# CityU-AIM-Group/SimT

Hardware: AMD Instinct MI355X
Metric: training images/sec at 768x768, DeepLabv2-R101+SimT (higher is better)
Workload: dtype bf16; 1 GPU; DeepLabv2-ResNet101 + SimT(C=19,K=3) full training iteration, batch=4/GPU, 768x768, bf16, 1xMI355X; global_batch=4, inputs=resident in HBM (see h2d_inclusive of a --full run for the PCIe-inclusive rate)

## Files before the change

### simt_amd/csrc/bn_pool.hip

```cpp
#include "common.h"

template <int NJ>
__device__ __forceinline__ void part_colsum8(const float* part, int nblk, int C, int c0, double* out , double (*red)[8][NJ]) {
  const int cl = threadIdx.x & 7, r = threadIdx.x >> 3;
  const int c = c0 + cl;
  double s[NJ];
#pragma unroll
  for (int j = 0; j < NJ; ++j) s[j] = 0.0;
  if (c < C) {
    int b = r;
    for (; b + 96 < nblk; b += 128) {
      float v[4][NJ];
#pragma unroll
      for (int u = 0; u < 4; ++u)
#pragma unroll
        for (int j = 0; j < NJ; ++j) v[u][j] = part[((long)(b + 32 * u) * NJ + j) * C + c];
#pragma unroll
      for (int u = 0; u < 4; ++u)
#pragma unroll
        for (int j = 0; j < NJ; ++j) s[j] += (double)v[u][j];
    }
    for (; b < nblk; b += 32)
#pragma unroll
      for (int j = 0; j < NJ; ++j) s[j] += (double)part[((long)b * NJ + j) * C + c];
// ... 308 lines not shown
      gr[u] = *(const uint2*)(dzb + ou);
      yr[u] = *(const uint2*)(yb + ou);
      if (MM == 1) zr[u] = *(const uint2*)(zb + ou);
      if (MM == 3) bb[u] = (unsigned)((const unsigned char*)zb)[ou >> 4] >> ((ou >> 1) & 4u);
    }
#pragma unroll
    for (int u = 0; u < UN; ++u) {
      const unsigned ou = o0 + u * Sb;
      if (ou >= nb) break;
      float g[4], yv[4];
      unpack4(gr[u], g);
      unpack4(yr[u], yv);
      if (MM == 1) {
        float zv[4];
        unpack4(zr[u], zv);
#pragma unroll
        for (int e = 0; e < 4; ++e) g[e] = zv[e] > 0.f ? g[e] : 0.f;
      } else if (MM == 2) {
#pragma unroll
        for (int e = 0; e < 4; ++e) g[e] = (yv[e] * sc[e] + sh[e]) > 0.f ? g[e] : 0.f;
      } else if (MM == 3) {
#pragma unroll
        for (int e = 0; e < 4; ++e) g[e] = ((bb[u] >> e) & 1u) ? g[e] : 0.f;
      }
      float o[4];
#pragma unroll
      for (int e = 0; e < 4; ++e) o[e] = sc[e] * (g[e] - c1[e] - ((yv[e] - mu[e]) * rs[e]) * c2[e]);
      *(uint2*)(dyb + ou) = make_uint2(pack_bf16x2(o[0], o[1]), pack_bf16x2(o[2], o[3]));
      if (gout) *(uint2*)(gb + ou) = make_uint2(pack_bf16x2(g[0], g[1]), pack_bf16x2(g[2], g[3]));
    }
  }
}

static inline int bn_bwd_rows_per_block(long M, int C) {
  int rpar = 256 / (C / 8);
  long target_blocks = 512;
  long rpb = (M + target_blocks - 1) / target_blocks;
  rpb = ((rpb + rpar - 1) / rpar) * rpar;
  if (rpb < rpar * 4) rpb = rpar * 4;
  return (int)rpb;
}

extern "C" int simt_bn_bwd_nblk(long M, int C) {
  int rpb = bn_bwd_rows_per_block(M, C);
  return (int)((M + rpb - 1) / rpb);
}

extern "C" int simt_bn_bwd(const simt_bn_bwd_desc* d, simt_stream_t stream) {
  SIMT_CHECK(d && d->dz && d->y && d->mean && d->rstd && d->scale && d->part && d->coef && d->dy);
  SIMT_CHECK(d->C % 8 == 0 && d->C / 8 <= 256 && 256 % (d->C / 8) == 0);
  SIMT_CHECK((d->mask_mode != 1 && d->mask_mode != 3) || d->z);
  SIMT_CHECK(d->mask_mode != 2 || d->shift);
  SIMT_CHECK(!d->y2 || (d->mean2 && d->rstd2 && d->scale2 && d->dy2));
  hipStream_t st = (hipStream_t)stream;
  const int rpb = bn_bwd_rows_per_block(d->M, d->C);
  const int nblk = d->reduce_done_nblk > 0 ? d->reduce_done_nblk : (int)((d->M + rpb - 1) / rpb);
  const long nvec = d->M * (d->C / 8);
  if (d->reduce_done_nblk > 0) {
    SIMT_CHECK(!d->y2);
  } else if (d->dtype == SIMT_BF16) {
    hipLaunchKernelGGL(bn_bwd_reduce_kernel<bf16_t>, dim3(nblk), dim3(256), 0, st, (const bf16_t*)d->dz,
                       (const bf16_t*)d->z, (const bf16_t*)d->y, d->mean, d->rstd, d->scale, d->shift,
                       (const bf16_t*)d->y2, d->mean2, d->rstd2, d->part, d->M, d->C, rpb, d->mask_mode);
  } else {
    hipLaunchKernelGGL(bn_bwd_reduce_kernel<float>, dim3(nblk), dim3(256), 0, st, (const float*)d->dz,
                       (const float*)d->z, (const float*)d->y, d->mean, d->rstd, d->scale, d->shift,
                       (const float*)d->y2, d->mean2, d->rstd2, d->part, d->M, d->C, rpb, d->mask_mode);
  }
  SIMT_LAUNCH_CHECK();
  hipLaunchKernelGGL(bn_bwd_finalize_kernel, dim3((d->C + 7) / 8), dim3(256), 0, st, d->part, nblk, d->C, d->M, d->coef,
                     d->dgamma, d->dbeta, d->dgamma2, d->dbeta2);
  SIMT_LAUNCH_CHECK();
  if (SIMT_BNB_APPLY4 && d->dtype == SIMT_BF16 && !d->y2 && nvec * 16 < (1l << 31)) {
#ifndef SIMT_BNB_APPLY4_CAP
#define SIMT_BNB_APPLY4_CAP 4096
#endif
    long gl = (nvec * 2 + 256l * SIMT_BNB_APPLY4_UN - 1) / (256l * SIMT_BNB_APPLY4_UN);
    int g4 = (int)(gl > SIMT_BNB_APPLY4_CAP ? SIMT_BNB_APPLY4_CAP : gl < 1 ? 1 : gl);
    if (d->C / 4 > 256) g4 = (g4 + 1) & ~1;
#define SIMT_BNB4(MM) hipLaunchKernelGGL(bn_bwd_apply4_kernel<MM>, dim3(g4), dim3(256), 0, st, (const bf16_t*)d->dz, (const bf16_t*)d->z, (const bf16_t*)d->y, \
                                         d->mean, d->rstd, d->scale, d->shift, d->coef, (bf16_t*)d->dy, (bf16_t*)d->gout, nvec * 2, d->C)
    if (d->mask_mode == 3) SIMT_BNB4(3); else if (d->mask_mode == 2) SIMT_BNB4(2); else if (d->mask_mode == 1) SIMT_BNB4(1); else SIMT_BNB4(0);
#undef SIMT_BNB4
  } else if (d->dtype == SIMT_BF16) {
    hipLaunchKernelGGL(bn_bwd_apply_kernel<bf16_t>, dim3(ew_grid(nvec)), dim3(256), 0, st, (const bf16_t*)d->dz,
                       (const bf16_t*)d->z, (const bf16_t*)d->y, d->mean, d->rstd, d->scale, d->shift, d->coef,
                       (const bf16_t*)d->y2, d->mean2, d->rstd2, d->scale2, (bf16_t*)d->dy, (bf16_t*)d->dy2,
                       (bf16_t*)d->gout, nvec, d->C, d->mask_mode);
  } else {
    hipLaunchKernelGGL(bn_bwd_apply_kernel<float>, dim3(ew_grid(nvec)), dim3(256), 0, st, (const float*)d->dz,
                       (const float*)d->z, (const float*)d->y, d->mean, d->rstd, d->scale, d->shift, d->coef,
                       (const float*)d->y2, d->mean2, d->rstd2, d->scale2, (float*)d->dy, (float*)d->dy2,
                       (float*)d->gout, nvec, d->C, d->mask_mode);
  }
  SIMT_LAUNCH_CHECK();
  return SIMT_OK;
}

template <typename T, int KHC, int KWC>
__global__ void im2col_stem_kernel(const float* x, T* A, int B, int Cin, int H, int W, int Ho, int Wo, int KHr, int KWr,
                                   int stride, int pad, int ldk, long nvec) {
  const int KH = KHC > 0 ? KHC : KHr, KW = KWC > 0 ? KWC : KWr;
  const int vpr = ldk >> 3;
  const int K = Cin * KH * KW;
  for (long i = (long)blockIdx.x * blockDim.x + threadIdx.x; i < nvec; i += (long)gridDim.x * blockDim.x) {
    int kv = (int)(i % vpr) << 3;
    long m = i / vpr;
    int ox = (int)(m % Wo);
    long t = m / Wo;
    int oy = (int)(t % Ho);
    int b = (int)(t / Ho);
    const int iy0 = oy * stride - pad, ix0 = ox * stride - pad;
    const float* xb = x + (long)b * Cin * H * W;
    float v[8];
#pragma unroll
    for (int e = 0; e < 8; ++e) {
      int k = kv + e;
      float val = 0.f;
      if (k < K) {
        int ci = k / (KH * KW);
        int rs = k - ci * KH * KW;
        int r = rs / KW, s = rs - r * KW;
        int iy = iy0 + r, ix = ix0 + s;
        if (iy >= 0 && iy < H && ix >= 0 && ix < W) val = xb[((long)ci * H + iy) * W + ix];
      }
      v[e] = val;
    }
    store8(A + i * 8, v);
  }
}

template <typename T>
static void launch_im2col(const float* x, T* A, int B, int Cin, int H, int W, int Ho, int Wo, int KH, int KW, int stride, int pad,
                          int ldk, long nvec, hipStream_t st) {
  const dim3 grid(ew_grid(nvec)), blk(256);
  if (KH == 7 && KW == 7)
    hipLaunchKernelGGL((im2col_stem_kernel<T, 7, 7>), grid, blk, 0, st, x, A, B, Cin, H, W, Ho, Wo, KH, KW, stride, pad, ldk, nvec);
  else if (KH == 3 && KW == 3)
    hipLaunchKernelGGL((im2col_stem_kernel<T, 3, 3>), grid, blk, 0, st, x, A, B, Cin, H, W, Ho, Wo, KH, KW, stride, pad, ldk, nvec);
  else
    hipLaunchKernelGGL((im2col_stem_kernel<T, 0, 0>), grid, blk, 0, st, x, A, B, Cin, H, W, Ho, Wo, KH, KW, stride, pad, ldk, nvec);
}

extern "C" int simt_im2col_stem(const float* x, void* A, int B, int Cin, int H, int W, int Ho, int Wo, int KH, int KW,
                                int stride, int pad, int ldk, int dtype, simt_stream_t stream) {
  SIMT_CHECK(x && A && ldk % 8 == 0 && ldk >= Cin * KH * KW);
  long nvec = (long)B * Ho * Wo * (ldk / 8);
  if (dtype == SIMT_BF16) launch_im2col<bf16_t>(x, (bf16_t*)A, B, Cin, H, W, Ho, Wo, KH, KW, stride, pad, ldk, nvec, (hipStream_t)stream);
  else launch_im2col<float>(x, (float*)A, B, Cin, H, W, Ho, Wo, KH, KW, stride, pad, ldk, nvec, (hipStream_t)stream);
  SIMT_LAUNCH_CHECK();
  return SIMT_OK;
}

template <typename T>
__global__ void bn_relu_maxpool_kernel(const T* y, const float* scale, const float* shift, T* p, unsigned char* idx,
                                       int B, int H, int W, int C, int Hp, int Wp, long nvec) {
  const int vpr = C >> 3;
  for (long i = (long)blockIdx.x * blockDim.x + threadIdx.x; i < nvec; i += (long)gridDim.x * blockDim.x) {
    int c = (int)(i % vpr) << 3;
    long m = i / vpr;
    int px = (int)(m % Wp);
    long t = m / Wp;
    int py = (int)(t % Hp);
    int b = (int)(t / Hp);
    float sc[8], sh[8], best[8];
    int bi[8];
    load8(scale + c, sc);
    load8(shift + c, sh);
#pragma unroll
    for (int e = 0; e < 8; ++e) { best[e] = -INFINITY; bi[e] = 0; }
    bool first = true;
    for (int r = 0; r < 3; ++r) {
      int iy = py * 2 - 1 + r;
      if (iy < 0 || iy >= H) continue;
      for (int s = 0; s < 3; ++s) {
        int ix = px * 2 - 1 + s;
        if (ix < 0 || ix >= W) continue;
        float v[8];
        load8(y + (((long)b * H + iy) * W + ix) * C + c, v);
#pragma unroll
        for (int e = 0; e < 8; ++e) {
          float a = v[e] * sc[e] + sh[e];
          a = a > 0.f ? a : 0.f;
          if (first || a > best[e] || a != a) { best[e] = a; bi[e] = r * 3 + s; }
        }
        first = false;
      }
    }
    store8(p + i * 8, best);
    unsigned long long packed = 0;
#pragma unroll
    for (int e = 0; e < 8; ++e) packed |= (unsigned long long)(bi[e] & 0xff) << (8 * e);
    *(unsigned long long*)(idx + i * 8) = packed;
  }
}

template <typename T>
__global__ void maxpool_bwd_kernel(const T* dp, const unsigned char* idx, T* da, int B, int H, int W, int C, int Hp,
                                   int Wp, long nvec) {
  const int vpr = C >> 3;
  for (long i = (long)blockIdx.x * blockDim.x + threadIdx.x; i < nvec; i += (long)gridDim.x * blockDim.x) {
    int c = (int)(i % vpr) << 3;
    long m = i / vpr;
    int ix = (int)(m % W);
    long t = m / W;
    int iy = (int)(t % H);
    int b = (int)(t / H);
    float acc[8];
#pragma unroll
    for (int e = 0; e < 8; ++e) acc[e] = 0.f;
    int py0 = iy >> 1, px0 = ix >> 1;
    for (int py = py0; py <= ((iy + 1) >> 1); ++py) {
      if (py >= Hp) continue;
      int r = iy - (py * 2 - 1);
      if (r < 0 || r > 2) continue;
      for (int px = px0; px <= ((ix + 1) >> 1); ++px) {
        if (px >= Wp) continue;
        int s = ix - (px * 2 - 1);
        if (s < 0 || s > 2) continue;
        long o = (((long)b * Hp + py) * Wp + px) * C + c;
        unsigned long long packed = *(const unsigned long long*)(idx + o);
        float g[8];
        load8(dp + o, g);
        int want = r * 3 + s;
#pragma unroll
        for (int e = 0; e < 8; ++e)
          if ((int)((packed >> (8 * e)) & 0xff) == want) acc[e] += g[e];
      }
    }
    store8(da + i * 8, acc);
  }
}

extern "C" int simt_bn_relu_maxpool(const void* y, const float* scale, const float* shift, void* p, unsigned char* idx,
                                    int B, int H, int W, int C, int Hp, int Wp, int dtype, simt_stream_t stream) {
  SIMT_CHECK(y && scale && shift && p && idx && C % 8 == 0);
  long nvec = (long)B * Hp * Wp * (C / 8);
  if (dtype == SIMT_BF16)
    hipLaunchKernelGGL(bn_relu_maxpool_kernel<bf16_t>, dim3(ew_grid(nvec)), dim3(256), 0, (hipStream_t)stream,
                       (const bf16_t*)y, scale, shift, (bf16_t*)p, idx, B, H, W, C, Hp, Wp, nvec);
  else
    hipLaunchKernelGGL(bn_relu_maxpool_kernel<float>, dim3(ew_grid(nvec)), dim3(256), 0, (hipStream_t)stream,
                       (const float*)y, scale, shift, (float*)p, idx, B, H, W, C, Hp, Wp, nvec);
  SIMT_LAUNCH_CHECK();
  return SIMT_OK;
}

extern "C" int simt_maxpool_bwd(const void* dp, const unsigned char* idx, void* da, int B, int H, int W, int C, int Hp,
                                int Wp, int dtype, simt_stream_t stream) {
  SIMT_CHECK(dp && idx && da && C % 8 == 0);
  long nvec = (long)B * H * W * (C / 8);
  if (dtype == SIMT_BF16)
    hipLaunchKernelGGL(maxpool_bwd_kernel<bf16_t>, dim3(ew_grid(nvec)), dim3(256), 0, (hipStream_t)stream,
                       (const bf16_t*)dp, idx, (bf16_t*)da, B, H, W, C, Hp, Wp, nvec);
  else
    hipLaunchKernelGGL(maxpool_bwd_kernel<float>, dim3(ew_grid(nvec)), dim3(256), 0, (hipStream_t)stream, (const float*)dp,
                       idx, (float*)da, B, H, W, C, Hp, Wp, nvec);
  SIMT_LAUNCH_CHECK();
  return SIMT_OK;
}

__device__ __forceinline__ long long frag_offset(long long row, long long kcol, int nt16) {
  const long long kt = kcol >> 6, s = (kcol >> 5) & 1, kq = (kcol >> 3) & 3, e = kcol & 7;
  const long long lane = (row & 15) | (kq << 4);
  return ((((kt * nt16 + (row >> 4)) * 2 + s) * 64 + lane) << 3) + e;
}
template <typename T>
__global__ void pack_weight_kernel(const float* w, T* dst, int Cout, int Cin, int RS, int row_off, int tap_off, long ldk,
                                   int Ck, int mode, const float* cscale, long total) {
  for (long i = (long)blockIdx.x * blockDim.x + threadIdx.x; i < total; i += (long)gridDim.x * blockDim.x) {
    int t = (int)(i % RS);
    long r = i / RS;
    int ci = (int)(r % Cin);
    int co = (int)(r / Cin);
    float v = w[i];
    if (cscale) v *= cscale[co];
    const int lm = mode & 0xff, nt16 = mode >> 8;
    const long row = lm == 0 ? (long)(row_off + co) : lm == 1 ? (long)ci : (long)(tap_off + t) * Ck + row_off + co;
    const long kcol = lm == 0 ? (long)(tap_off + t) * Cin + ci : lm == 1 ? (long)(tap_off + t) * Ck + row_off + co : (long)ci;
    const long o = nt16 ? (long)frag_offset(row, kcol, nt16) : row * ldk + kcol;
    Elem<T>::st(dst + o, v);
  }
}

extern "C" int simt_pack_weight(const float* w, void* dst, int Cout, int Cin, int RS, int row_off, int tap_off, long ldk,
                                int Ck, int mode, const float* cscale, int dtype, simt_stream_t stream) {
  SIMT_CHECK(w && dst && Cout > 0 && Cin > 0 && RS > 0);
  long total = (long)Cout * Cin * RS;
  if (dtype == SIMT_BF16)
    hipLaunchKernelGGL(pack_weight_kernel<bf16_t>, dim3(ew_grid(total)), dim3(256), 0, (hipStream_t)stream, w, (bf16_t*)dst,
                       Cout, Cin, RS, row_off, tap_off, ldk, Ck, mode, cscale, total);
  else
    hipLaunchKernelGGL(pack_weight_kernel<float>, dim3(ew_grid(total)), dim3(256), 0, (hipStream_t)stream, w, (float*)dst,
                       Cout, Cin, RS, row_off, tap_off, ldk, Ck, mode, cscale, total);
  SIMT_LAUNCH_CHECK();
  return SIMT_OK;
}

struct PackJob {
  const float* w;
  void* dst;
  const float* cscale;
  long long ldk, total;
  int Cout, Cin, RS, row_off, tap_off, Ck, mode, dtype;
};
template <int RSC>
__device__ __forceinline__ void pack_tile(const PackJob& j, int tidx, float* tile) {
  const int ntc = (j.Cin + 31) >> 5;
  const int co0 = (tidx / ntc) << 5, ci0 = (tidx % ntc) << 5;
  const int RS = RSC > 0 ? RSC : j.RS;
  const int nci = min(32, j.Cin - ci0), nco = min(32, j.Cout - co0);
  for (int tb = 0; tb < RS; tb += 9) {
    const int nt = min(9, RS - tb);
    __syncthreads();
    const int per_co = nci * RS;
    for (int e = threadIdx.x; e < nco * per_co; e += 256) {
      const int co_l = e / per_co, rem = e - co_l * per_co;
      const int ci_l = rem / RS, t = rem - ci_l * RS;
      if (t < tb || t >= tb + nt) continue;
      float v = j.w[((long long)(co0 + co_l) * j.Cin + ci0) * RS + rem];
      if (j.cscale) v *= j.cscale[co0 + co_l];
      tile[((t - tb) * 32 + co_l) * 33 + ci_l] = v;
    }
    __syncthreads();
    for (int e = threadIdx.x; e < nt * 32 * 32; e += 256) {
      const int t = e >> 10;
      int co_l, ci_l;
      const int lm = j.mode & 0xff, nt16 = j.mode >> 8;
      if (lm == 1) { co_l = e & 31; ci_l = (e >> 5) & 31; } else { ci_l = e & 31; co_l = (e >> 5) & 31; }
      if (co_l >= nco || ci_l >= nci) continue;
      const float v = tile[(t * 32 + co_l) * 33 + ci_l];
      const int co = co0 + co_l, ci = ci0 + ci_l, tt = j.tap_off + tb + t;
      const long long row = lm == 0 ? (long long)(j.row_off + co) : lm == 1 ? (long long)ci : (long long)tt * j.Ck + j.row_off + co;
      const long long kcol = lm == 0 ? (long long)tt * j.Cin + ci : lm == 1 ? (long long)tt * j.Ck + j.row_off + co : (long long)ci;
      const long long o = nt16 ? frag_offset(row, kcol, nt16) : row * j.ldk + kcol;
      if (j.dtype == SIMT_BF16) ((bf16_t*)j.dst)[o] = f2bf(v); else ((float*)j.dst)[o] = v;
    }
  }
}
__global__ __launch_bounds__(256) void pack_weight_multi_kernel(const PackJob* jobs, const int* chunks, int ) {
  __shared__ float tile[9 * 32 * 33];
  const PackJob j = jobs[chunks[2 * blockIdx.x]];
  const int tidx = chunks[2 * blockIdx.x + 1];
  if (j.RS == 1) pack_tile<1>(j, tidx, tile);
  else if (j.RS == 9) pack_tile<9>(j, tidx, tile);
  else pack_tile<0>(j, tidx, tile);
}
extern "C" int simt_pack_weight_multi(const void* jobs, const void* chunks, int nchunks, int chunk, simt_stream_t stream) {
  SIMT_CHECK(jobs && chunks && nchunks > 0);
  hipLaunchKernelGGL(pack_weight_multi_kernel, dim3(nchunks), dim3(256), 0, (hipStream_t)stream, (const PackJob*)jobs,
                     (const int*)chunks, chunk);
  SIMT_LAUNCH_CHECK();
  return SIMT_OK;
}

__global__ void bn_fold_kernel(const float* gamma, const float* beta, const float* rm, const float* rv, float eps,
                               float* scale, float* shift, int C) {
  int c = blockIdx.x * blockDim.x + threadIdx.x;
  if (c >= C) return;
  float sc = gamma[c] / sqrtf(rv[c] + eps);
  scale[c] = sc;
  shift[c] = beta[c] - rm[c] * sc;
}
extern "C" int simt_bn_fold(const float* gamma, const float* beta, const float* rm, const float* rv, float eps,
                            float* scale, float* shift, int C, simt_stream_t stream) {
  SIMT_CHECK(gamma && beta && rm && rv && scale && shift);
  hipLaunchKernelGGL(bn_fold_kernel, dim3((C + 63) / 64), dim3(64), 0, (hipStream_t)stream, gamma, beta, rm, rv, eps,
                     scale, shift, C);
  SIMT_LAUNCH_CHECK();
  return SIMT_OK;
}

template <typename T>
__global__ void scatter_stride_kernel(const T* src, T* dx, int B, int H, int W, int C, int Ho, int Wo, int stride,
                                      long nvec) {
  const int vpr = C >> 3;
  for (long i = (long)blockIdx.x * blockDim.x + threadIdx.x; i < nvec; i += (long)gridDim.x * blockDim.x) {
    int c = (int)(i % vpr) << 3;
    long m = i / vpr;
    int ix = (int)(m % W);
    long t = m / W;
    int iy = (int)(t % H);
    int b = (int)(t / H);
    float v[8];
#pragma unroll
    for (int e = 0; e < 8; ++e) v[e] = 0.f;
    if (iy % stride == 0 && ix % stride == 0) {
      int oy = iy / stride, ox = ix / stride;
      if (oy < Ho && ox < Wo) load8(src + (((long)b * Ho + oy) * Wo + ox) * C + c, v);
    }
    store8(dx + i * 8, v);
  }
}
extern "C" int simt_scatter_stride(const void* src, void* dx, int B, int H, int W, int C, int Ho, int Wo, int stride,
                                   int dtype, simt_stream_t stream) {
  SIMT_CHECK(src && dx && C % 8 == 0);
  long nvec = (long)B * H * W * (C / 8);
  if (dtype == SIMT_BF16)
    hipLaunchKernelGGL(scatter_stride_kernel<bf16_t>, dim3(ew_grid(nvec)), dim3(256), 0, (hipStream_t)stream,
                       (const bf16_t*)src, (bf16_t*)dx, B, H, W, C, Ho, Wo, stride, nvec);
  else
    hipLaunchKernelGGL(scatter_stride_kernel<float>, dim3(ew_grid(nvec)), dim3(256), 0, (hipStream_t)stream,
                       (const float*)src, (float*)dx, B, H, W, C, Ho, Wo, stride, nvec);
  SIMT_LAUNCH_CHECK();
  return SIMT_OK;
}

#define COLSUM_G 128
__device__ double g_colsum_ws[COLSUM_G * 64];

template <typename T>
__global__ __launch_bounds__(256) void colsum_partial_kernel(const T* src, long M, int ld, int C) {
  __shared__ double red[4][64];
  const int c = threadIdx.x & 63, lr = threadIdx.x >> 6;
  long rows = (M + COLSUM_G - 1) / COLSUM_G;
  long m0 = (long)blockIdx.x * rows, m1 = m0 + rows;
  if (m1 > M) m1 = M;
  double s = 0.0;
  if (c < C)
    for (long m = m0 + lr; m < m1; m += 4) s += (double)Elem<T>::ld(src + m * ld + c);
  red[lr][c] = s;
  __syncthreads();
  if (lr == 0) g_colsum_ws[blockIdx.x * 64 + c] = red[0][c] + red[1][c] + red[2][c] + red[3][c];
}
__global__ void colsum_final_kernel(float* out, int C, int accumulate) {
  int c = threadIdx.x;
  if (c >= C) return;
  double t = 0.0;
  for (int b = 0; b < COLSUM_G; ++b) t += g_colsum_ws[b * 64 + c];
  out[c] = accumulate ? out[c] + (float)t : (float)t;
}
extern "C" int simt_colsum(const void* src, float* out, long M, int ld, int C, int accumulate, int dtype,
                           simt_stream_t stream) {
  SIMT_CHECK(src && out && C <= 64);
  if (dtype == SIMT_BF16)
    hipLaunchKernelGGL(colsum_partial_kernel<bf16_t>, dim3(COLSUM_G), dim3(256), 0, (hipStream_t)stream, (const bf16_t*)src, M, ld, C);
  else
    hipLaunchKernelGGL(colsum_partial_kernel<float>, dim3(COLSUM_G), dim3(256), 0, (hipStream_t)stream, (const float*)src, M, ld, C);
  SIMT_LAUNCH_CHECK();
  hipLaunchKernelGGL(colsum_final_kernel, dim3(1), dim3(64), 0, (hipStream_t)stream, out, C, accumulate);
  SIMT_LAUNCH_CHECK();
  return SIMT_OK;
}

template <typename T>
__global__ void maxpool2_kernel(const T* y, T* p, unsigned char* idx, int B, int H, int W, int C, int Hp, int Wp, long nvec) {
  const int vpr = C >> 3;
  for (long i = (long)blockIdx.x * blockDim.x + threadIdx.x; i < nvec; i += (long)gridDim.x * blockDim.x) {
    int c = (int)(i % vpr) << 3;
    long m = i / vpr;
    int px = (int)(m % Wp);
    long t = m / Wp;
    int py = (int)(t % Hp);
    int b = (int)(t / Hp);
    float best[8];
    int bi[8];
#pragma unroll
    for (int e = 0; e < 8; ++e) { best[e] = -INFINITY; bi[e] = 0; }
#pragma unroll
    for (int r = 0; r < 2; ++r)
#pragma unroll
      for (int s = 0; s < 2; ++s) {
        float v[8];
        load8(y + (((long)b * H + py * 2 + r) * W + px * 2 + s) * C + c, v);
#pragma unroll
        for (int e = 0; e < 8; ++e)
          if ((r == 0 && s == 0) || v[e] > best[e] || v[e] != v[e]) { best[e] = v[e]; bi[e] = r * 2 + s; }
      }
    store8(p + i * 8, best);
    unsigned long long packed = 0;
#pragma unroll
    for (int e = 0; e < 8; ++e) packed |= (unsigned long long)bi[e] << (8 * e);
    *(unsigned long long*)(idx + i * 8) = packed;
  }
}

template <typename T>
__global__ void maxpool2_bwd_kernel(const T* dp, const unsigned char* idx, const T* y, T* da, int B, int H, int W, int C, int Hp,
                                    int Wp, long nvec) {
  const int vpr = C >> 3;
  for (long i = (long)blockIdx.x * blockDim.x + threadIdx.x; i < nvec; i += (long)gridDim.x * blockDim.x) {
    int c = (int)(i % vpr) << 3;
    long m = i / vpr;
    int ix = (int)(m % W);
    long t = m / W;
    int iy = (int)(t % H);
    int b = (int)(t / H);
    float out[8];
#pragma unroll
    for (int e = 0; e < 8; ++e) out[e] = 0.f;
    const int py = iy >> 1, px = ix >> 1;
    if (py < Hp && px < Wp) {
      long o = (((long)b * Hp + py) * Wp + px) * C + c;
      unsigned long long packed = *(const unsigned long long*)(idx + o);
      float g[8], yv[8];
      load8(dp + o, g);
      load8(y + i * 8, yv);
      const int want = (iy & 1) * 2 + (ix & 1);
#pragma unroll
      for (int e = 0; e < 8; ++e)
        if ((int)((packed >> (8 * e)) & 0xff) == want && (!y || yv[e] > 0.f)) out[e] = g[e];
    }
    store8(da + i * 8, out);
  }
}

extern "C" int simt_maxpool2(const void* y, void* p, unsigned char* idx, int B, int H, int W, int C, int dtype, simt_stream_t stream) {
  SIMT_CHECK(y && p && idx && C % 8 == 0);
  const int Hp = H / 2, Wp = W / 2;
  long nvec = (long)B * Hp * Wp * (C / 8);
  if (dtype == SIMT_BF16)
    hipLaunchKernelGGL(maxpool2_kernel<bf16_t>, dim3(ew_grid(nvec)), dim3(256), 0, (hipStream_t)stream, (const bf16_t*)y, (bf16_t*)p,
                       idx, B, H, W, C, Hp, Wp, nvec);
  else
    hipLaunchKernelGGL(maxpool2_kernel<float>, dim3(ew_grid(nvec)), dim3(256), 0, (hipStream_t)stream, (const float*)y, (float*)p, idx,
                       B, H, W, C, Hp, Wp, nvec);
  SIMT_LAUNCH_CHECK();
  return SIMT_OK;
}

extern "C" int simt_maxpool2_bwd(const void* dp, const unsigned char* idx, const void* y, void* da, int B, int H, int W, int C, int dtype,
                                 simt_stream_t stream) {
  SIMT_CHECK(dp && idx && y && da && C % 8 == 0);
  const int Hp = H / 2, Wp = W / 2;
  long nvec = (long)B * H * W * (C / 8);
  if (dtype == SIMT_BF16)
    hipLaunchKernelGGL(maxpool2_bwd_kernel<bf16_t>, dim3(ew_grid(nvec)), dim3(256), 0, (hipStream_t)stream, (const bf16_t*)dp, idx,
                       (const bf16_t*)y, (bf16_t*)da, B, H, W, C, Hp, Wp, nvec);
  else
    hipLaunchKernelGGL(maxpool2_bwd_kernel<float>, dim3(ew_grid(nvec)), dim3(256), 0, (hipStream_t)stream, (const float*)dp, idx,
                       (const float*)y, (float*)da, B, H, W, C, Hp, Wp, nvec);
  SIMT_LAUNCH_CHECK();
  return SIMT_OK;
}

#define COLSUMW_G 1024
#define COLSUMW_MAXC 2048
__device__ float g_colsumw_ws[COLSUMW_G * COLSUMW_MAXC];
template <typename T>
__global__ __launch_bounds__(256) void colsum_wide_partial_kernel(const T* src, long M, int ld, int C, int rows_per_block) {
  __shared__ float red[256][8 + 1];
  const int vpr = C >> 3;
  const int rpar = 256 / vpr;
  const int tid = threadIdx.x, vc = tid % vpr, rl = tid / vpr;
  float s[8];
#pragma unroll
  for (int e = 0; e < 8; ++e) s[e] = 0.f;
  const long r0 = (long)blockIdx.x * rows_per_block;
  long r1 = r0 + rows_per_block;
  if (r1 > M) r1 = M;
  if (rl < rpar) {
    long r = r0 + rl;
    for (; r + 3 * rpar < r1; r += 4 * rpar) {
      float v[4][8];
#pragma unroll
      for (int u = 0; u < 4; ++u) load8(src + (r + u * rpar) * ld + (vc << 3), v[u]);
#pragma unroll
      for (int u = 0; u < 4; ++u)
#pragma unroll
        for (int e = 0; e < 8; ++e) s[e] += v[u][e];
    }
    for (; r < r1; r += rpar) {
      float v[8];
      load8(src + r * ld + (vc << 3), v);
#pragma unroll
      for (int e = 0; e < 8; ++e) s[e] += v[e];
    }
  }
#pragma unroll
  for (int e = 0; e < 8; ++e) red[tid][e] = s[e];
  __syncthreads();
  for (int cc = tid; cc < C; cc += 256) {
    const int v = cc >> 3, e = cc & 7;
// ... 29 lines not shown
```

### simt_amd/csrc/head_expand.hip

```cpp
#include "common.h"

struct TapArgs {
  const void* src;
  const float* bias;
  void* dst;
  int B, H, W, Q, QP, lds, ldd, ntaps;
  long M;
  short dy[SIMT_MAX_TAPS], dx[SIMT_MAX_TAPS];
};

__global__ __launch_bounds__(256) void tap_gather_sum_kernel(TapArgs a) {
  const int nq = a.QP >> 2;
  const long total = a.M * nq;
  const float* P = (const float*)a.src;
  float* y = (float*)a.dst;
  for (long idx = (long)blockIdx.x * blockDim.x + threadIdx.x; idx < total; idx += (long)gridDim.x * blockDim.x) {
    const int q = (int)(idx % nq);
    const long m = idx / nq;
    const int ox = (int)(m % a.W);
    const long t2 = m / a.W;
    const int oy = (int)(t2 % a.H);
    float4 acc = make_float4(0.f, 0.f, 0.f, 0.f);
    if (a.bias) {
      const int c = q * 4;
      acc.x = c + 0 < a.Q ? a.bias[c + 0] : 0.f;
      acc.y = c + 1 < a.Q ? a.bias[c + 1] : 0.f;
      acc.z = c + 2 < a.Q ? a.bias[c + 2] : 0.f;
      acc.w = c + 3 < a.Q ? a.bias[c + 3] : 0.f;
    }
    for (int t = 0; t < a.ntaps; ++t) {
      const int iy = oy + a.dy[t], ix = ox + a.dx[t];
      if (iy < 0 || iy >= a.H || ix < 0 || ix >= a.W) continue;
      const float4 v = *(const float4*)(P + (m + (long)a.dy[t] * a.W + a.dx[t]) * a.lds + t * a.QP + q * 4);
      acc.x += v.x; acc.y += v.y; acc.z += v.z; acc.w += v.w;
    }
    *(float4*)(y + m * a.ldd + q * 4) = acc;
  }
}

__global__ __launch_bounds__(256) void tap_scatter_kernel(TapArgs a) {
  const int ng = a.QP >> 3;
  const long total = a.M * a.ntaps * ng;
  const bf16_t* d = (const bf16_t*)a.src;
  bf16_t* G = (bf16_t*)a.dst;
  for (long idx = (long)blockIdx.x * blockDim.x + threadIdx.x; idx < total; idx += (long)gridDim.x * blockDim.x) {
    const int g = (int)(idx % ng);
    long r = idx / ng;
    const int t = (int)(r % a.ntaps);
    const long m = r / a.ntaps;
    const int ox = (int)(m % a.W);
    const int oy = (int)((m / a.W) % a.H);
    const int iy = oy - a.dy[t], ix = ox - a.dx[t];
    uint4 v = make_uint4(0u, 0u, 0u, 0u);
    if (iy >= 0 && iy < a.H && ix >= 0 && ix < a.W)
      v = *(const uint4*)(d + (m - ((long)a.dy[t] * a.W + a.dx[t])) * a.lds + g * 8);
    st_out16(G + m * a.ldd + t * a.QP + g * 8, v);
  }
}

static int tap_grid(long total) {
  long g = (total + 255) / 256;
  if (g > 256 * 16) g = 256 * 16;
  return (int)(g < 1 ? 1 : g);
}

extern "C" int simt_tap_gather_sum(const simt_tap_desc* d, simt_stream_t stream) {
  SIMT_CHECK(d && d->src && d->dst && d->ntaps >= 1 && d->ntaps <= SIMT_MAX_TAPS);
  SIMT_CHECK(d->QP % 4 == 0 && d->lds % 4 == 0 && d->ldd % 4 == 0 && d->QP <= d->ldd && d->ntaps * d->QP <= d->lds);
  TapArgs a;
  a.src = d->src; a.bias = d->bias; a.dst = d->dst; a.B = d->B; a.H = d->H; a.W = d->W; a.Q = d->Q; a.QP = d->QP;
  a.lds = d->lds; a.ldd = d->ldd; a.ntaps = d->ntaps; a.M = (long)d->B * d->H * d->W;
  for (int i = 0; i < SIMT_MAX_TAPS; ++i) { a.dy[i] = d->dy[i]; a.dx[i] = d->dx[i]; }
  hipLaunchKernelGGL(tap_gather_sum_kernel, dim3(tap_grid(a.M * (a.QP / 4))), dim3(256), 0, (hipStream_t)stream, a);
  SIMT_LAUNCH_CHECK();
  return SIMT_OK;
}

extern "C" int simt_tap_scatter(const simt_tap_desc* d, simt_stream_t stream) {
  SIMT_CHECK(d && d->src && d->dst && d->ntaps >= 1 && d->ntaps <= SIMT_MAX_TAPS);
  SIMT_CHECK(d->QP % 8 == 0 && d->lds % 8 == 0 && d->ldd % 8 == 0 && d->QP <= d->lds && d->ntaps * d->QP <= d->ldd);
  TapArgs a;
  a.src = d->src; a.bias = nullptr; a.dst = d->dst; a.B = d->B; a.H = d->H; a.W = d->W; a.Q = d->Q; a.QP = d->QP;
  a.lds = d->lds; a.ldd = d->ldd; a.ntaps = d->ntaps; a.M = (long)d->B * d->H * d->W;
  for (int i = 0; i < SIMT_MAX_TAPS; ++i) { a.dy[i] = d->dy[i]; a.dx[i] = d->dx[i]; }
  hipLaunchKernelGGL(tap_scatter_kernel, dim3(tap_grid(a.M * a.ntaps * (a.QP / 8))), dim3(256), 0, (hipStream_t)stream, a);
  SIMT_LAUNCH_CHECK();
  return SIMT_OK;
}
```

Measured before the change: 173.9 images/s.

## Restructure maxpool, weight packing, colsum and tap kernels for row reuse and vectorization

The fused BN-ReLU-maxpool forward now walks strips of output rows per thread and reuses the overlapping input row between windows. The maxpool backward becomes a gather that produces each 2x2 input block from the four pooled windows it touches. Weight packing converts to the target dtype inside LDS and writes 16-byte vectors, with a direct path for 1x1 weights. The column-sum loop and the tap gather loop are unrolled to keep more loads in flight, and both tap kernels now use a 2D row-based grid instead of div/mod index math. Together these aim to cut redundant loads and index arithmetic in small memory-bound kernels, at the cost of more code and different grid shapes, including a very small y-dimension for the scatter kernel.

```diff
diff --git a/simt_amd/csrc/bn_pool.hip b/simt_amd/csrc/bn_pool.hip
--- a/simt_amd/csrc/bn_pool.hip
+++ b/simt_amd/csrc/bn_pool.hip
@@ -484,96 +484,168 @@
   return SIMT_OK;
 }
 
-template <typename T>
-__global__ void bn_relu_maxpool_kernel(const T* y, const float* scale, const float* shift, T* p, unsigned char* idx,
-                                       int B, int H, int W, int C, int Hp, int Wp, long nvec) {
+#define POOL_ROWS 4
+template <typename T>
+__global__ __launch_bounds__(256) void bn_relu_maxpool_kernel(const T* y, const float* scale, const float* shift, T* p, unsigned char* idx,
+                                                              int B, int H, int W, int C, int Hp, int Wp, int nstrips) {
   const int vpr = C >> 3;
-  for (long i = (long)blockIdx.x * blockDim.x + threadIdx.x; i < nvec; i += (long)gridDim.x * blockDim.x) {
-    int c = (int)(i % vpr) << 3;
-    long m = i / vpr;
-    int px = (int)(m % Wp);
-    long t = m / Wp;
-    int py = (int)(t % Hp);
-    int b = (int)(t / Hp);
-    float sc[8], sh[8], best[8];
-    int bi[8];
-    load8(scale + c, sc);
-    load8(shift + c, sh);
-#pragma unroll
-    for (int e = 0; e < 8; ++e) { best[e] = -INFINITY; bi[e] = 0; }
+  const int item = blockIdx.y * 256 + threadIdx.x;
+  const int px = item / vpr, c = (item - px * vpr) << 3;
+  if (px >= Wp) return;
+  const int b = blockIdx.x / nstrips, py0 = (blockIdx.x - b * nstrips) * POOL_ROWS;
+  float sc[8], sh[8];
+  load8(scale + c, sc);
+  load8(shift + c, sh);
+  const int ix0 = px * 2 - 1;
+  bool okx[3];
+#pragma unroll
+  for (int s = 0; s < 3; ++s) okx[s] = ix0 + s >= 0 && ix0 + s < W;
+  const T* yb = y + (long)b * H * W * C + c;
+  float keep[3][8];
+  for (int k = 0; k < POOL_ROWS; ++k) {
+    const int py = py0 + k;
+    if (py >= Hp) break;
+    const int iy0 = py * 2 - 1;
+    Raw8<T> raw[3][3];
+#pragma unroll
+    for (int r = 0; r < 3; ++r) {
+      const int iy = iy0 + r;
+      if ((r == 0 && k > 0) || iy < 0 || iy >= H) continue;
+#pragma unroll
+      for (int s = 0; s < 3; ++s)
+        if (okx[s]) raw8_load(yb + ((long)iy * W + ix0 + s) * C, raw[r][s]);
+    }
+    float best[8];
+    unsigned long long packed = 0;
+#pragma unroll
+    for (int e = 0; e < 8; ++e) best[e] = -INFINITY;
     bool first = true;
+#pragma unroll
     for (int r = 0; r < 3; ++r) {
-      int iy = py * 2 - 1 + r;
+      const int iy = iy0 + r;
       if (iy < 0 || iy >= H) continue;
+#pragma unroll
       for (int s = 0; s < 3; ++s) {
-        int ix = px * 2 - 1 + s;
-        if (ix < 0 || ix >= W) continue;
-        float v[8];
-        load8(y + (((long)b * H + iy) * W + ix) * C + c, v);
+        if (!okx[s]) continue;
+        float a[8];
+        if (r == 0 && k > 0) {
+#pragma unroll
+          for (int e = 0; e < 8; ++e) a[e] = keep[s][e];
+        } else {
+          float v[8];
+          raw8_unpack(raw[r][s], v);
+#pragma unroll
+          for (int e = 0; e < 8; ++e) {
+            const float t = __builtin_fmaf(v[e], sc[e], sh[e]);
+            a[e] = t > 0.f ? t : 0.f;
+          }
+        }
 #pragma unroll
         for (int e = 0; e < 8; ++e) {
-          float a = v[e] * sc[e] + sh[e];
-          a = a > 0.f ? a : 0.f;
-          if (first || a > best[e] || a != a) { best[e] = a; bi[e] = r * 3 + s; }
+          if (first || a[e] > best[e] || a[e] != a[e]) {
+            best[e] = a[e];
+            packed = (packed & ~(0xffull << (8 * e))) | ((unsigned long long)(r * 3 + s) << (8 * e));
+          }
+          if (r == 2) keep[s][e] = a[e];
         }
         first = false;
       }
     }
-    store8(p + i * 8, best);
-    unsigned long long packed = 0;
-#pragma unroll
-    for (int e = 0; e < 8; ++e) packed |= (unsigned long long)(bi[e] & 0xff) << (8 * e);
-    *(unsigned long long*)(idx + i * 8) = packed;
-  }
-}
-
-template <typename T>
-__global__ void maxpool_bwd_kernel(const T* dp, const unsigned char* idx, T* da, int B, int H, int W, int C, int Hp,
-                                   int Wp, long nvec) {
+    const long o = ((((long)b * Hp + py) * Wp + px) * vpr << 3) + c;
+    store8(p + o, best);
+    *(unsigned long long*)(idx + o) = packed;
+  }
+}
+
+template <typename T> struct PoolWin { Raw8<T> g; unsigned long long k; };
+template <typename T>
+__device__ __forceinline__ void pool_win_load(const T* dp, const unsigned char* idx, long o, PoolWin<T>& w) {
+  raw8_load(dp + o, w.g);
+  w.k = *(const unsigned long long*)(idx + o);
+}
+template <typename T>
+__device__ __forceinline__ void pool_win_add(const PoolWin<T>& w, int want, float* acc) {
+  float g[8];
+  raw8_unpack(w.g, g);
+#pragma unroll
+  for (int e = 0; e < 8; ++e)
+    if ((int)((w.k >> (8 * e)) & 0xff) == want) acc[e] += g[e];
+}
+template <typename T>
+__global__ __launch_bounds__(256) void maxpool_bwd_kernel(const T* dp, const unsigned char* idx, T* da, int B, int H, int W, int C, int Hp,
+                                                          int Wp, int nstrips) {
   const int vpr = C >> 3;
-  for (long i = (long)blockIdx.x * blockDim.x + threadIdx.x; i < nvec; i += (long)gridDim.x * blockDim.x) {
-    int c = (int)(i % vpr) << 3;
-    long m = i / vpr;
-    int ix = (int)(m % W);
-    long t = m / W;
-    int iy = (int)(t % H);
-    int b = (int)(t / H);
+  const int item = blockIdx.y * 256 + threadIdx.x;
+  const int px = item / vpr, c = (item - px * vpr) << 3;
+  if (px * 2 >= W) return;
+  const int b = blockIdx.x / nstrips, py0 = (blockIdx.x - b * nstrips) * POOL_ROWS;
+  const bool x1 = px * 2 + 1 < W;
+  const bool wx0 = px < Wp, wx1 = px + 1 < Wp;
+  const long pb = (long)b * Hp;
+  PoolWin<T> cur[2], nxt[2];
+  for (int k = 0; k < POOL_ROWS; ++k) {
+    const int py = py0 + k;
+    if (py * 2 >= H) break;
+    const bool y1 = py * 2 + 1 < H, wy0 = py < Hp, wy1 = py + 1 < Hp;
+    if (k == 0 && wy0) {
+      if (wx0) pool_win_load(dp, idx, (((pb + py) * Wp + px) * vpr << 3) + c, cur[0]);
+      if (wx1) pool_win_load(dp, idx, (((pb + py) * Wp + px + 1) * vpr << 3) + c, cur[1]);
+    }
+    if (wy1) {
+      if (wx0) pool_win_load(dp, idx, (((pb + py + 1) * Wp + px) * vpr << 3) + c, nxt[0]);
+      if (wx1) pool_win_load(dp, idx, (((pb + py + 1) * Wp + px + 1) * vpr << 3) + c, nxt[1]);
+    }
+    const bool w00 = wy0 && wx0, w01 = wy0 && wx1, w10 = wy1 && wx0, w11 = wy1 && wx1;
     float acc[8];
+    T* o0 = da + ((((long)b * H + py * 2) * W + px * 2) * vpr << 3) + c;
 #pragma unroll
     for (int e = 0; e < 8; ++e) acc[e] = 0.f;
-    int py0 = iy >> 1, px0 = ix >> 1;
-    for (int py = py0; py <= ((iy + 1) >> 1); ++py) {
-      if (py >= Hp) continue;
-      int r = iy - (py * 2 - 1);
-      if (r < 0 || r > 2) continue;
-      for (int px = px0; px <= ((ix + 1) >> 1); ++px) {
-        if (px >= Wp) continue;
-        int s = ix - (px * 2 - 1);
-        if (s < 0 || s > 2) continue;
-        long o = (((long)b * Hp + py) * Wp + px) * C + c;
-        unsigned long long packed = *(const unsigned long long*)(idx + o);
-        float g[8];
-        load8(dp + o, g);
-        int want = r * 3 + s;
-#pragma unroll
-        for (int e = 0; e < 8; ++e)
-          if ((int)((packed >> (8 * e)) & 0xff) == want) acc[e] += g[e];
+    if (w00) pool_win_add(cur[0], 4, acc);
+    store8(o0, acc);
+    if (x1) {
+#pragma unroll
+      for (int e = 0; e < 8; ++e) acc[e] = 0.f;
+      if (w00) pool_win_add(cur[0], 5, acc);
+      if (w01) pool_win_add(cur[1], 3, acc);
+      store8(o0 + C, acc);
+    }
+    if (y1) {
+#pragma unroll
+      for (int e = 0; e < 8; ++e) acc[e] = 0.f;
+      if (w00) pool_win_add(cur[0], 7, acc);
+      if (w10) pool_win_add(nxt[0], 1, acc);
+      store8(o0 + (long)W * C, acc);
+      if (x1) {
+#pragma unroll
+        for (int e = 0; e < 8; ++e) acc[e] = 0.f;
+        if (w00) pool_win_add(cur[0], 8, acc);
+        if (w01) pool_win_add(cur[1], 6, acc);
+        if (w10) pool_win_add(nxt[0], 2, acc);
+        if (w11) pool_win_add(nxt[1], 0, acc);
+        store8(o0 + (long)W * C + C, acc);
       }
     }
-    store8(da + i * 8, acc);
-  }
+    cur[0] = nxt[0];
+    cur[1] = nxt[1];
+  }
+}
+
+static dim3 pool_grid(int B, int rows, int cols, int C, int* nstrips) {
+  *nstrips = (rows + POOL_ROWS - 1) / POOL_ROWS;
+  return dim3((unsigned)(B * *nstrips), (unsigned)(((long)cols * (C / 8) + 255) / 256));
 }
 
 extern "C" int simt_bn_relu_maxpool(const void* y, const float* scale, const float* shift, void* p, unsigned char* idx,
                                     int B, int H, int W, int C, int Hp, int Wp, int dtype, simt_stream_t stream) {
   SIMT_CHECK(y && scale && shift && p && idx && C % 8 == 0);
-  long nvec = (long)B * Hp * Wp * (C / 8);
+  int nstrips;
+  const dim3 grid = pool_grid(B, Hp, Wp, C, &nstrips);
   if (dtype == SIMT_BF16)
-    hipLaunchKernelGGL(bn_relu_maxpool_kernel<bf16_t>, dim3(ew_grid(nvec)), dim3(256), 0, (hipStream_t)stream,
-                       (const bf16_t*)y, scale, shift, (bf16_t*)p, idx, B, H, W, C, Hp, Wp, nvec);
+    hipLaunchKernelGGL(bn_relu_maxpool_kernel<bf16_t>, grid, dim3(256), 0, (hipStream_t)stream,
+                       (const bf16_t*)y, scale, shift, (bf16_t*)p, idx, B, H, W, C, Hp, Wp, nstrips);
   else
-    hipLaunchKernelGGL(bn_relu_maxpool_kernel<float>, dim3(ew_grid(nvec)), dim3(256), 0, (hipStream_t)stream,
-                       (const float*)y, scale, shift, (float*)p, idx, B, H, W, C, Hp, Wp, nvec);
+    hipLaunchKernelGGL(bn_relu_maxpool_kernel<float>, grid, dim3(256), 0, (hipStream_t)stream,
+                       (const float*)y, scale, shift, (float*)p, idx, B, H, W, C, Hp, Wp, nstrips);
   SIMT_LAUNCH_CHECK();
   return SIMT_OK;
 }
@@ -581,13 +653,14 @@
 extern "C" int simt_maxpool_bwd(const void* dp, const unsigned char* idx, void* da, int B, int H, int W, int C, int Hp,
                                 int Wp, int dtype, simt_stream_t stream) {
   SIMT_CHECK(dp && idx && da && C % 8 == 0);
-  long nvec = (long)B * H * W * (C / 8);
+  int nstrips;
+  const dim3 grid = pool_grid(B, (H + 1) / 2, (W + 1) / 2, C, &nstrips);
   if (dtype == SIMT_BF16)
-    hipLaunchKernelGGL(maxpool_bwd_kernel<bf16_t>, dim3(ew_grid(nvec)), dim3(256), 0, (hipStream_t)stream,
-                       (const bf16_t*)dp, idx, (bf16_t*)da, B, H, W, C, Hp, Wp, nvec);
+    hipLaunchKernelGGL(maxpool_bwd_kernel<bf16_t>, grid, dim3(256), 0, (hipStream_t)stream,
+                       (const bf16_t*)dp, idx, (bf16_t*)da, B, H, W, C, Hp, Wp, nstrips);
   else
-    hipLaunchKernelGGL(maxpool_bwd_kernel<float>, dim3(ew_grid(nvec)), dim3(256), 0, (hipStream_t)stream, (const float*)dp,
-                       idx, (float*)da, B, H, W, C, Hp, Wp, nvec);
+    hipLaunchKernelGGL(maxpool_bwd_kernel<float>, grid, dim3(256), 0, (hipStream_t)stream, (const float*)dp,
+                       idx, (float*)da, B, H, W, C, Hp, Wp, nstrips);
   SIMT_LAUNCH_CHECK();
   return SIMT_OK;
 }
@@ -636,47 +709,122 @@
   long long ldk, total;
   int Cout, Cin, RS, row_off, tap_off, Ck, mode, dtype;
 };
-template <int RSC>
-__device__ __forceinline__ void pack_tile(const PackJob& j, int tidx, float* tile) {
+template <typename E> struct PackT;
+template <> struct PackT<bf16_t> {
+  static constexpr int VEC = 8, TS = 9;
+  static __device__ __forceinline__ bf16_t cvt(float v) { return f2bf(v); }
+  static __device__ __forceinline__ uint32_t word(const float* v, int w) { return (uint32_t)f2bf(v[2 * w]) | ((uint32_t)f2bf(v[2 * w + 1]) << 16); }
+  static __device__ __forceinline__ bf16_t get(uint32_t w, int i) { return (bf16_t)(w >> (16 * (i & 1))); }
+};
+template <> struct PackT<float> {
+  static constexpr int VEC = 4, TS = 4;
+  static __device__ __forceinline__ float cvt(float v) { return v; }
+  static __device__ __forceinline__ uint32_t word(const float* v, int w) { return __float_as_uint(v[w]); }
+  static __device__ __forceinline__ float get(uint32_t w, int) { return __uint_as_float(w); }
+};
+#define PACK_LDS_BYTES 23552
+
+__device__ __forceinline__ void pack_ld4(const float* p, int n, bool vec, float* x) {
+  if (vec && n >= 4) {
+    const float4 v = *(const float4*)p;
+    x[0] = v.x; x[1] = v.y; x[2] = v.z; x[3] = v.w;
+  } else {
+#pragma unroll
+    for (int i = 0; i < 4; ++i) x[i] = i < n ? p[i] : 0.f;
+  }
+}
+template <typename E>
+__device__ __forceinline__ void pack_st(const PackJob& j, long long row, long long kcol0, int nv, const uint4& v) {
+  constexpr int VEC = PackT<E>::VEC;
+  const int nt16 = j.mode >> 8;
+  E* dst = (E*)j.dst;
+  const long long o = row * j.ldk + kcol0;
+  if (!nt16 && nv == VEC && (((uintptr_t)(dst + o)) & 15) == 0) {
+    *(uint4*)(dst + o) = v;
+    return;
+  }
+  const uint32_t w[4] = {v.x, v.y, v.z, v.w};
+#pragma unroll
+  for (int i = 0; i < VEC; ++i)
+    if (i < nv) dst[nt16 ? frag_offset(row, kcol0 + i, nt16) : o + i] = PackT<E>::get(w[i * (int)sizeof(E) / 4], i);
+}
+
+template <int RSC, typename E>
+__device__ __forceinline__ void pack_tile(const PackJob& j, int tidx, unsigned char* smem) {
+  constexpr int VEC = PackT<E>::VEC, TS = PackT<E>::TS, NG = 32 / VEC;
+  constexpr int PITCH = 32 + VEC, PLANE = 32 * PITCH + VEC;
+  E* tile = (E*)smem;
   const int ntc = (j.Cin + 31) >> 5;
   const int co0 = (tidx / ntc) << 5, ci0 = (tidx % ntc) << 5;
   const int RS = RSC > 0 ? RSC : j.RS;
   const int nci = min(32, j.Cin - ci0), nco = min(32, j.Cout - co0);
-  for (int tb = 0; tb < RS; tb += 9) {
-    const int nt = min(9, RS - tb);
+  const int lm = j.mode & 0xff, nt16 = j.mode >> 8;
+  const int L = nci * RS;
+  const bool vsrc = (((uintptr_t)j.w) & 15) == 0 && ((j.Cin * RS) & 3) == 0;
+  if (RSC == 1 && lm == 0 && nt16 == 0) {
+    const int co_l = threadIdx.x / NG, ci_l = (threadIdx.x % NG) * VEC;
+    if (co_l >= nco || ci_l >= nci) return;
+    const int nv = min(VEC, nci - ci_l);
+    const float* p = j.w + (long long)(co0 + co_l) * j.Cin + ci0 + ci_l;
+    const float cs = j.cscale ? j.cscale[co0 + co_l] : 1.f;
+    float x[VEC];
+#pragma unroll
+    for (int h = 0; h < VEC; h += 4) pack_ld4(p + h, nv - h, vsrc, x + h);
+#pragma unroll
+    for (int i = 0; i < VEC; ++i) x[i] = j.cscale ? x[i] * cs : x[i];
+    const uint4 v = make_uint4(PackT<E>::word(x, 0), PackT<E>::word(x, 1), PackT<E>::word(x, 2), PackT<E>::word(x, 3));
+    pack_st<E>(j, (long long)(j.row_off + co0 + co_l), (long long)j.tap_off * j.Cin + ci0 + ci_l, nv, v);
+    return;
+  }
+  const int co_r = threadIdx.x >> 3, q0 = threadIdx.x & 7;
+  const int nq = (L + 3) >> 2;
+  for (int tb = 0; tb < RS; tb += TS) {
+    const int nt = min(TS, RS - tb);
     __syncthreads();
-    const int per_co = nci * RS;
-    for (int e = threadIdx.x; e < nco * per_co; e += 256) {
-      const int co_l = e / per_co, rem = e - co_l * per_co;
-      const int ci_l = rem / RS, t = rem - ci_l * RS;
-      if (t < tb || t >= tb + nt) continue;
-      float v = j.w[((long long)(co0 + co_l) * j.Cin + ci0) * RS + rem];
-      if (j.cscale) v *= j.cscale[co0 + co_l];
-      tile[((t - tb) * 32 + co_l) * 33 + ci_l] = v;
+    if (co_r < nco) {
+      const float* run = j.w + ((long long)(co0 + co_r) * j.Cin + ci0) * RS;
+      const float cs = j.cscale ? j.cscale[co0 + co_r] : 1.f;
+      for (int q = q0; q < nq; q += 8) {
+        float x[4];
+        pack_ld4(run + 4 * q, L - 4 * q, vsrc, x);
+#pragma unroll
+        for (int i = 0; i < 4; ++i) {
+          const int rem = 4 * q + i;
+          const int ci_l = rem / RS, t = rem - ci_l * RS;
+          if (rem >= L || t < tb || t >= tb + nt) continue;
+          const float v = j.cscale ? x[i] * cs : x[i];
+          tile[(t - tb) * PLANE + (lm == 1 ? ci_l * PITCH + co_r : co_r * PITCH + ci_l)] = PackT<E>::cvt(v);
+        }
+      }
     }
     __syncthreads();
-    for (int e = threadIdx.x; e < nt * 32 * 32; e += 256) {
-      const int t = e >> 10;
-      int co_l, ci_l;
-      const int lm = j.mode & 0xff, nt16 = j.mode >> 8;
-      if (lm == 1) { co_l = e & 31; ci_l = (e >> 5) & 31; } else { ci_l = e & 31; co_l = (e >> 5) & 31; }
-      if (co_l >= nco || ci_l >= nci) continue;
-      const float v = tile[(t * 32 + co_l) * 33 + ci_l];
-      const int co = co0 + co_l, ci = ci0 + ci_l, tt = j.tap_off + tb + t;
-      const long long row = lm == 0 ? (long long)(j.row_off + co) : lm == 1 ? (long long)ci : (long long)tt * j.Ck + j.row_off + co;
-      const long long kcol = lm == 0 ? (long long)tt * j.Cin + ci : lm == 1 ? (long long)tt * j.Ck + j.row_off + co : (long long)ci;
-      const long long o = nt16 ? frag_offset(row, kcol, nt16) : row * j.ldk + kcol;
-      if (j.dtype == SIMT_BF16) ((bf16_t*)j.dst)[o] = f2bf(v); else ((float*)j.dst)[o] = v;
-    }
-  }
+    for (int e = threadIdx.x; e < nt * 32 * NG; e += 256) {
+      const int g = e % NG, r_l = (e / NG) & 31, t = e / (NG * 32);
+      const int tt = j.tap_off + tb + t;
+      const int nrow = lm == 1 ? nci : nco, ncol = lm == 1 ? nco : nci;
+      if (r_l >= nrow || g * VEC >= ncol) continue;
+      const int nv = min(VEC, ncol - g * VEC);
+      const uint4 v = *(const uint4*)(tile + t * PLANE + r_l * PITCH + g * VEC);
+      long long row, kcol;
+      if (lm == 0) { row = j.row_off + co0 + r_l; kcol = (long long)tt * j.Cin + ci0 + g * VEC; }
+      else if (lm == 1) { row = ci0 + r_l; kcol = (long long)tt * j.Ck + j.row_off + co0 + g * VEC; }
+      else { row = (long long)tt * j.Ck + j.row_off + co0 + r_l; kcol = ci0 + g * VEC; }
+      pack_st<E>(j, row, kcol, nv, v);
+    }
+  }
+}
+template <typename E>
+__device__ __forceinline__ void pack_tile_rs(const PackJob& j, int tidx, unsigned char* smem) {
+  if (j.RS == 1) pack_tile<1, E>(j, tidx, smem);
+  else if (j.RS == 9) pack_tile<9, E>(j, tidx, smem);
+  else pack_tile<0, E>(j, tidx, smem);
 }
 __global__ __launch_bounds__(256) void pack_weight_multi_kernel(const PackJob* jobs, const int* chunks, int ) {
-  __shared__ float tile[9 * 32 * 33];
+  __shared__ __attribute__((aligned(16))) unsigned char smem[PACK_LDS_BYTES];
   const PackJob j = jobs[chunks[2 * blockIdx.x]];
   const int tidx = chunks[2 * blockIdx.x + 1];
-  if (j.RS == 1) pack_tile<1>(j, tidx, tile);
-  else if (j.RS == 9) pack_tile<9>(j, tidx, tile);
-  else pack_tile<0>(j, tidx, tile);
+  if (j.dtype == SIMT_BF16) pack_tile_rs<bf16_t>(j, tidx, smem);
+  else pack_tile_rs<float>(j, tidx, smem);
 }
 extern "C" int simt_pack_weight_multi(const void* jobs, const void* chunks, int nchunks, int chunk, simt_stream_t stream) {
   SIMT_CHECK(jobs && chunks && nchunks > 0);
@@ -749,8 +897,17 @@
   long m0 = (long)blockIdx.x * rows, m1 = m0 + rows;
   if (m1 > M) m1 = M;
   double s = 0.0;
-  if (c < C)
-    for (long m = m0 + lr; m < m1; m += 4) s += (double)Elem<T>::ld(src + m * ld + c);
+  if (c < C) {
+    long m = m0 + lr;
+    for (; m + 28 < m1; m += 32) {
+      float v[8];
+#pragma unroll
+      for (int u = 0; u < 8; ++u) v[u] = Elem<T>::ld(src + (m + 4 * u) * ld + c);
+#pragma unroll
+      for (int u = 0; u < 8; ++u) s += (double)v[u];
+    }
+    for (; m < m1; m += 4) s += (double)Elem<T>::ld(src + m * ld + c);
+  }
   red[lr][c] = s;
   __syncthreads();
   if (lr == 0) g_colsum_ws[blockIdx.x * 64 + c] = red[0][c] + red[1][c] + red[2][c] + red[3][c];
diff --git a/simt_amd/csrc/head_expand.hip b/simt_amd/csrc/head_expand.hip
--- a/simt_amd/csrc/head_expand.hip
+++ b/simt_amd/csrc/head_expand.hip
@@ -9,17 +9,15 @@
   short dy[SIMT_MAX_TAPS], dx[SIMT_MAX_TAPS];
 };
 
+
+#define TAP_BATCH 6
 __global__ __launch_bounds__(256) void tap_gather_sum_kernel(TapArgs a) {
   const int nq = a.QP >> 2;
-  const long total = a.M * nq;
-  const float* P = (const float*)a.src;
-  float* y = (float*)a.dst;
-  for (long idx = (long)blockIdx.x * blockDim.x + threadIdx.x; idx < total; idx += (long)gridDim.x * blockDim.x) {
-    const int q = (int)(idx % nq);
-    const long m = idx / nq;
-    const int ox = (int)(m % a.W);
-    const long t2 = m / a.W;
-    const int oy = (int)(t2 % a.H);
+  const int oy = (int)(blockIdx.x % (unsigned)a.H);
+  for (int item = blockIdx.y * 256 + threadIdx.x; item < a.W * nq; item += gridDim.y * 256) {
+    const int ox = item / nq, q = item - ox * nq;
+    const long m = (long)blockIdx.x * a.W + ox;
+    const float* P = (const float*)a.src + m * a.lds + q * 4;
     float4 acc = make_float4(0.f, 0.f, 0.f, 0.f);
     if (a.bias) {
       const int c = q * 4;
@@ -28,40 +26,59 @@
       acc.z = c + 2 < a.Q ? a.bias[c + 2] : 0.f;
       acc.w = c + 3 < a.Q ? a.bias[c + 3] : 0.f;
     }
-    for (int t = 0; t < a.ntaps; ++t) {
-      const int iy = oy + a.dy[t], ix = ox + a.dx[t];
-      if (iy < 0 || iy >= a.H || ix < 0 || ix >= a.W) continue;
-      const float4 v = *(const float4*)(P + (m + (long)a.dy[t] * a.W + a.dx[t]) * a.lds + t * a.QP + q * 4);
-      acc.x += v.x; acc.y += v.y; acc.z += v.z; acc.w += v.w;
+    for (int t0 = 0; t0 < a.ntaps; t0 += TAP_BATCH) {
+      float4 v[TAP_BATCH];
+      bool ok[TAP_BATCH];
+#pragma unroll
+      for (int k = 0; k < TAP_BATCH; ++k) {
+        const int t = t0 + k;
+        ok[k] = false;
+        if (t < a.ntaps) {
+          const int dy = a.dy[t], dx = a.dx[t];
+          const int iy = oy + dy, ix = ox + dx;
+          if (iy >= 0 && iy < a.H) {
+            ok[k] = ix >= 0 && ix < a.W;
+            if (ok[k]) v[k] = *(const float4*)(P + ((long)dy * a.W + dx) * a.lds + t * a.QP);
+          }
+        }
+      }
+#pragma unroll
+      for (int k = 0; k < TAP_BATCH; ++k)
+        if (ok[k]) { acc.x += v[k].x; acc.y += v[k].y; acc.z += v[k].z; acc.w += v[k].w; }
     }
-    *(float4*)(y + m * a.ldd + q * 4) = acc;
+    *(float4*)((float*)a.dst + m * a.ldd + q * 4) = acc;
   }
 }
 
 __global__ __launch_bounds__(256) void tap_scatter_kernel(TapArgs a) {
   const int ng = a.QP >> 3;
-  const long total = a.M * a.ntaps * ng;
+  const int per_px = a.ntaps * ng;
+  const int nitems = a.W * per_px;
+  const int oy = (int)(blockIdx.x % (unsigned)a.H);
+  const long m0 = (long)blockIdx.x * a.W;
   const bf16_t* d = (const bf16_t*)a.src;
   bf16_t* G = (bf16_t*)a.dst;
-  for (long idx = (long)blockIdx.x * blockDim.x + threadIdx.x; idx < total; idx += (long)gridDim.x * blockDim.x) {
-    const int g = (int)(idx % ng);
-    long r = idx / ng;
-    const int t = (int)(r % a.ntaps);
-    const long m = r / a.ntaps;
-    const int ox = (int)(m % a.W);
-    const int oy = (int)((m / a.W) % a.H);
-    const int iy = oy - a.dy[t], ix = ox - a.dx[t];
+  __shared__ short sdy[SIMT_MAX_TAPS], sdx[SIMT_MAX_TAPS];
+  for (int t = 0; t < a.ntaps; ++t)
+    if (threadIdx.x == 0) { sdy[t] = a.dy[t]; sdx[t] = a.dx[t]; }
+  __syncthreads();
+  for (int item = blockIdx.y * 256 + threadIdx.x; item < nitems; item += gridDim.y * 256) {
+    const int ox = item / per_px, c = item - ox * per_px;
+    const int t = c / ng, g = c - t * ng;
+    const int dy = sdy[t], dx = sdx[t];
+    const int iy = oy - dy, ix = ox - dx;
+    const long m = m0 + ox;
     uint4 v = make_uint4(0u, 0u, 0u, 0u);
     if (iy >= 0 && iy < a.H && ix >= 0 && ix < a.W)
-      v = *(const uint4*)(d + (m - ((long)a.dy[t] * a.W + a.dx[t])) * a.lds + g * 8);
+      v = *(const uint4*)(d + (m - ((long)dy * a.W + dx)) * a.lds + g * 8);
     st_out16(G + m * a.ldd + t * a.QP + g * 8, v);
   }
 }
 
-static int tap_grid(long total) {
-  long g = (total + 255) / 256;
-  if (g > 256 * 16) g = 256 * 16;
-  return (int)(g < 1 ? 1 : g);
+static unsigned tap_slices(long items, int cap) {
+  long g = (items + 255) / 256;
+  if (g > cap) g = cap;
+  return (unsigned)(g < 1 ? 1 : g);
 }
 
 extern "C" int simt_tap_gather_sum(const simt_tap_desc* d, simt_stream_t stream) {
@@ -71,7 +88,7 @@
   a.src = d->src; a.bias = d->bias; a.dst = d->dst; a.B = d->B; a.H = d->H; a.W = d->W; a.Q = d->Q; a.QP = d->QP;
   a.lds = d->lds; a.ldd = d->ldd; a.ntaps = d->ntaps; a.M = (long)d->B * d->H * d->W;
   for (int i = 0; i < SIMT_MAX_TAPS; ++i) { a.dy[i] = d->dy[i]; a.dx[i] = d->dx[i]; }
-  hipLaunchKernelGGL(tap_gather_sum_kernel, dim3(tap_grid(a.M * (a.QP / 4))), dim3(256), 0, (hipStream_t)stream, a);
+  hipLaunchKernelGGL(tap_gather_sum_kernel, dim3((unsigned)(a.B * a.H), tap_slices((long)a.W * (a.QP / 4), 65535)), dim3(256), 0, (hipStream_t)stream, a);
   SIMT_LAUNCH_CHECK();
   return SIMT_OK;
 }
@@ -83,7 +100,7 @@
   a.src = d->src; a.bias = nullptr; a.dst = d->dst; a.B = d->B; a.H = d->H; a.W = d->W; a.Q = d->Q; a.QP = d->QP;
   a.lds = d->lds; a.ldd = d->ldd; a.ntaps = d->ntaps; a.M = (long)d->B * d->H * d->W;
   for (int i = 0; i < SIMT_MAX_TAPS; ++i) { a.dy[i] = d->dy[i]; a.dx[i] = d->dx[i]; }
-  hipLaunchKernelGGL(tap_scatter_kernel, dim3(tap_grid(a.M * a.ntaps * (a.QP / 8))), dim3(256), 0, (hipStream_t)stream, a);
+  hipLaunchKernelGGL(tap_scatter_kernel, dim3((unsigned)(a.B * a.H), tap_slices((long)a.W * a.ntaps * (a.QP / 8), 4)), dim3(256), 0, (hipStream_t)stream, a);
   SIMT_LAUNCH_CHECK();
   return SIMT_OK;
 }
```

Result: no change. 175.4 images/s (median of 6 runs) (+0.9%).
